# theori-io/nrsc5

Hardware: NVIDIA H100
Metric: cu8 I/Q Msamples/s (higher is better)
Workload: dtype u8/int16/f32

## Files before the change

### nrsc5_b200/csrc/front.cuh

```cuda
#pragma once
#include "pids_crc.cuh"
#include "common.cuh"
#include "fft.cuh"
#include "viterbi_pack.cuh"

namespace nb {

constexpr int FRONT_THREADS = 1024;
constexpr int TEAMS = FRONT_THREADS / 128;
constexpr int MAXREF = 15;
constexpr int IN_BYTES = 4 * NSYM + 28 + 16 + 16;
constexpr int IN_STRIDE = 8704;
constexpr int ACQ_TILE = 4096;

__device__ int g_dbg;

__constant__ int c_compat_mode[64];
__constant__ unsigned c_pn80[3];
__constant__ short c_bp_tap[32];

__device__ __forceinline__ float2 cmulf(float2 a, float2 b)
{
    return make_float2(a.x * b.x - a.y * b.y, a.x * b.y + a.y * b.x);
}
// ... 18 lines not shown
{
    StreamState &st = p.st[s];
    if (st.state == ns) return;
    if (st.state == ST_FINE) log_reserve(p, d, s, REC_LOST_SYNC, 0);
    if (ns == ST_FINE) {
        float fo = (float)(((double)st.prev_angle - 2 * M_PI * st.cfo) * 744187.5 / (2 * M_PI * NFFT));
        uint8_t *w = log_reserve(p, d, s, REC_SYNC, 8);
        if (w) {
            reinterpret_cast<float *>(w)[0] = fo;
            reinterpret_cast<int *>(w)[1] = st.psmi;
        }
    }
    st.state = ns;
}

constexpr int DEMOD_RUN = 17;
constexpr int TEAM_SMEM = IN_STRIDE + NSYM * (int)sizeof(short2);
struct DemodSmem {
    float2 buf[TEAMS][TEAM_SMEM / sizeof(float2)];
    float2 symphase[TEAMS];
};
static_assert(FFT_SMEM_ELEMS * sizeof(float2) <= TEAM_SMEM && TEAM_SMEM % 16 == 0, "a team's FFT buffer");
static_assert(DEMOD_RUN * FFT_THREADS >= NSYM && DEMOD_RUN % 2 == 1, "a symbol's runs");
struct PrepSmem {
    uint32_t words[ACQ_TILE + 40];
    short2 ytile[ACQ_TILE + 32];
    float2 sums[NSYM];
    float red_mag[FRONT_THREADS];
    int red_idx[FRONT_THREADS];
    float2 red_v[FRONT_THREADS];
};
constexpr int ACQ1_RUN = 3;
constexpr int ACQ1_WORDS = (NSYM + 38 + 3 + 3) / 4 * 4;
static_assert(ACQ1_RUN * FRONT_THREADS >= NSYM + 31 && ACQ1_RUN % 2 == 1, "a tile's runs");
struct Acq1Smem {
    uint32_t words[2][ACQ1_WORDS];
    short2 ytile[NSYM + 32];
    float2 ring[2][NSYM];
    float2 sums[NSYM];
    float2 shape[NCP];
    float red_mag[FRONT_THREADS];
    int red_idx[FRONT_THREADS];
    float2 red_v[FRONT_THREADS];
};
struct PidsSmem {
    int8_t vit[PIDS_LEN * 3];
    uint2 dec[PIDS_LEN + 64];
};
constexpr int ZS = 32;
constexpr int EQ_LD = BLK + 1;
constexpr int EQ_MAXPART = 12;
constexpr int EQ_ROWS = 2 * EQ_MAXPART * (PW - 1);
struct SyncSmem {
    float2 zref[BLK][ZS];
    float phs[BLK][ZS];
    float2 eph[2 * MAXREF][BLK];
    float smag[2 * MAXREF];
    float cfq[2 * MAXREF];
    union {
        float2 eq[EQ_ROWS][EQ_LD];
        struct {
            int offs[76][22];
            int verdict[76];
            int winner;
        } srch;
    };
    float wred[FRONT_THREADS / 32][2];
    float fb_w[2][MAXREF], fb_xy[2][MAXREF + 1];
    float4 rowc[EQ_ROWS];
    int ref_ok[2 * MAXREF], ref_bc[2 * MAXREF], ref_psmi[2 * MAXREF];
    float mult[2];
    float angle;
    int do_search;
};
struct FrontSmem {
    float2 tw[FFT_TW];
    float2 nco[NSYM];
    union {
        DemodSmem demod;
        PrepSmem prep;
        Acq1Smem acq1;
        SyncSmem sync;
        PidsSmem pidsq[16];
    } u;
};

__device__ void pids_decode_warp(const DevPtrs &p, const EngineDims &d, int s, int e, PidsSmem &sm, int lane)
{
    const StreamState &st = p.st[s];
    const int bc = st.pids_bc[e];
    const int8_t *pmall = p.pm + (size_t)s * 16 * PM_BLOCK;
    const int8_t PMV[20] = { 10, 2, 18, 6, 14, 8, 16, 0, 12, 4, 11, 3, 19, 7, 15, 9, 17, 1, 13, 5 };
    for (int o = lane; o < PIDS_LEN * 3; o += 32) {
        int8_t v = 0;
        if (o % 6 != 5) {
            unsigned i = (unsigned)bc * 200 + (unsigned)(o - o / 6);
            unsigned part = (unsigned)PMV[i % 20];
            unsigned block = i / 200;
            unsigned k = (i / 20) % 10 + P1_ENC / 320;
            unsigned row = (k * 11) % 32, col = (k * 11 + k / 288) % 36;
            v = pmall[(block * 32 + row) * 720 + part * 36 + col];
        }
        sm.vit[o] = v;
    }
    __syncwarp();
    const int l = lane & 15;
    VitHalf<false> vh;
    vh.init(l);
    vitc_run<false>(vh, sm.vit, PIDS_LEN, PIDS_LEN + 64, 0, PIDS_LEN + 64, 0, sm.dec, lane < 16, l);
    __syncwarp();
    int v = (short)(vh.E & 0xffff), state = 2 * l;
    const int w1 = (short)(vh.O & 0xffff);
    if (w1 > v) { v = w1; state = 2 * l + 1; }
    int v2 = (short)(vh.E >> 16), idx2 = 2 * l + 32;
    const int w3 = (short)(vh.O >> 16);
    if (w3 > v2) { v2 = w3; idx2 = 2 * l + 33; }
    if (v2 > v) { v = v2; state = idx2; }
#pragma unroll
    for (int o = 8; o; o >>= 1) {
        const int ov = __shfl_xor_sync(0xffffffffu, v, o, 16), oi = __shfl_xor_sync(0xffffffffu, state, o, 16);
        if (ov > v || (ov == v && oi < state)) { v = ov; state = oi; }
    }
    if (lane == 0) {
        uint8_t pk[10];
        for (int i = 0; i < 10; i++) pk[i] = 0;
        for (int q = PIDS_LEN + 63; q >= 0; q--) {
            if (q >= 32 && q < 32 + PIDS_LEN) {
                const int i = q - 32;
                const int bit = ((state >> 5) & 1) ^ (int)((c_pn80[i >> 5] >> (i & 31)) & 1u);
                pk[i >> 3] |= (uint8_t)(bit << (7 - (i & 7)));
// ... 373 lines not shown
        st.prev_angle = angle;
        sh_angle = angle;
    }
    __syncthreads();

    const int samperr = sh_samperr;
    const int adj = NSYM / 2 - samperr;
    if (adj != 0) {
        float *cp = p.cphase + (size_t)s * NFFT;
        for (int i = t; i < SIDE; i += FRONT_THREADS) {
            const int bl = LB0 + i, bu = UB1 - i;
            cp[bl] = (float)((double)cp[bl] - (double)(adj * (bl - NFFT / 2) * 2) * M_PI / NFFT);
            cp[bu] = (float)((double)cp[bu] - (double)(adj * (bu - NFFT / 2) * 2) * M_PI / NFFT);
        }
    }
    if (t == 0) {
        float angle = sh_angle;
        angle = (float)((double)angle - 2 * M_PI * st.cfo);
        const float pre = (float)(-adj) * angle / (float)NFFT;
        const float2 ph = cmulf(st.phase, cexp_j(pre));
        const float theta = angle / (float)NFFT;
        st.phase0 = ph;
        st.theta = theta;
        sh_theta = theta;
        st.blk_samperr = samperr;
        st.blk_state_in = state_in;
        double sn, cs;
        sincos((double)theta * (double)(NSYM * BLK), &sn, &cs);
        const float2 pe = cmulf(ph, make_float2((float)cs, (float)sn));
        const float nrm = sqrtf(pe.x * pe.x + pe.y * pe.y);
        st.phase = make_float2(pe.x / nrm, pe.y / nrm);
        uint8_t *w = log_reserve(p, d, s, REC_BLOCK, 32);
        if (w) {
            int *wi = reinterpret_cast<int *>(w);
            float *wf = reinterpret_cast<float *>(w);
            wi[0] = state_in; wi[1] = samperr; wf[2] = angle; wf[3] = ph.x; wf[4] = ph.y; wi[5] = st.cfo;
            wi[6] = (int)(unsigned)(st.start & 0xffffffffLL);
            wi[7] = (int)(st.start >> 32);
        }
    }
    __syncthreads();
    fill_nco(p, nco, sh_theta, t);
    __syncthreads();
    return true;
}

__device__ __forceinline__ float2 sample_q15(short2 h)
{
    const float sc = 1.0f / 32767.0f;
    return make_float2((float)h.x * sc, (float)h.y * -sc);
}

__device__ void front_demod(const DevPtrs &p, const EngineDims &d, int s, int sym, DemodSmem &sm, const float2 *nco,
                            const float2 *tw, int half, int tl, long long start, int samperr, float theta, float2 phase0)
{
    float2 *buf = sm.buf[half];
    uint8_t *in = reinterpret_cast<uint8_t *>(buf);
    const int bar = 1 + half;
    const long long base = start + samperr + (long long)NSYM * sym;
    const long long b0 = 4 * base - 28;
    const long long b0a = b0 & ~15LL;
    const int off = (int)(b0 - b0a);
    const uint8_t *iq = p.iq + (size_t)s * d.in_stride;
    bar_sync(bar);
    {
        const int nvec = (off + 4 * NSYM + 28 + 15) / 16;
        uint4 *dst = reinterpret_cast<uint4 *>(in);
        for (int v = tl; v < nvec; v += 128) {
            const long long a = b0a + 16LL * v;
            if (a >= 0) {
#if defined(NB_EMU)
                dst[v] = *reinterpret_cast<const uint4 *>(iq + a);
#else
                asm volatile("cp.async.cg.shared.global [%0], [%1], 16;" ::"r"((unsigned)__cvta_generic_to_shared(dst + v)), "l"(iq + a) : "memory");
#endif
            } else {
                dst[v] = make_uint4(0x7f7f7f7fu, 0x7f7f7f7fu, 0x7f7f7f7fu, 0x7f7f7f7fu);
            }
        }
#if !defined(NB_EMU)
        asm volatile("cp.async.commit_group;\n\tcp.async.wait_group 0;" ::: "memory");
#endif
    }
    if (tl == 0) {
        double sn, cs;
        sincos((double)theta * (double)(NSYM * sym), &sn, &cs);
        sm.symphase[half] = cmul(phase0, make_float2((float)cs, (float)sn));
    }
    bar_sync(bar);

    const uint32_t *sw = reinterpret_cast<const uint32_t *>(in + off);
    const short2 *y;
    if (d.cs16) {
        y = reinterpret_cast<const short2 *>(sw + 7);
    } else {
        short2 *yw = reinterpret_cast<short2 *>(in + IN_STRIDE);
        const int j0 = min(DEMOD_RUN * tl, NSYM - DEMOD_RUN);
        halfband_run<DEMOD_RUN>(sw + j0, yw + j0);
        y = yw;
        bar_sync(bar);
    }
    float2 v[16];
    v[0] = cmul(sample_q15(y[tl]), nco[tl]);
    if (tl < NCP) {
        const int j = NFFT + tl;
        v[0] = cadd(v[0], cmul(sample_q15(y[j]), nco[j]));
    }
#pragma unroll
    for (int n1 = 1; n1 < 16; n1++) {
        const int j = n1 * 128 + tl;
        v[n1] = cmul(sample_q15(y[j]), nco[j]);
    }
    bar_sync(bar);
    float2 out[2][8];
    fft2048_block<true>(v, out, buf, tw, tl, bar);
    const float2 sp = sm.symphase[half];

    float2 *dst = p.bins + ((size_t)s * BLK + sym) * NBINS;
#pragma unroll
    for (int h = 0; h < 2; h++) {
        const int q = tl + 128 * h;
        if (q >= 222) dst[q - 222] = cmul(out[h][5], sp);
        if (q <= 232) dst[q + 34] = cmul(out[h][6], sp);
        if (q >= 24) dst[q + 243] = cmul(out[h][1], sp);
        if (q <= 34) dst[q + 499] = cmul(out[h][2], sp);
    }
}

__device__ __forceinline__ int ref_bin(int slot)
{
    return slot < MAXREF ? LB0 + PW * slot : UB1 - PW * (slot - MAXREF);
}

__device__ __forceinline__ float atan2_short(float y, float x)
{
    const float ax = fabsf(x), ay = fabsf(y);
    const float mx = fmaxf(ax, ay), mn = fminf(ax, ay);
    const float t = mx > 0.f ? __fdividef(mn, mx) : 0.f;
    const float z = t * t;
    float p = 0.0028340641874819994f;
    p = __fmaf_rn(p, z, -0.016005029901862144f);
    p = __fmaf_rn(p, z, 0.042587608098983765f);
    p = __fmaf_rn(p, z, -0.07495445758104324f);
    p = __fmaf_rn(p, z, 0.10636754333972931f);
    p = __fmaf_rn(p, z, -0.14202570915222168f);
    p = __fmaf_rn(p, z, 0.19992484152317047f);
    p = __fmaf_rn(p, z, -0.3333306610584259f);
    p = __fmaf_rn(p, z, 1.0f);
    float r = p * t;
    if (ay > ax) r = 1.57079637f - r;
    if (x < 0.f) r = 3.14159274f - r;
    return copysignf(r, y);
}

__device__ __forceinline__ void costas_row(float2 *z, float *phs, int zs, float &cfreq, float &cphase, int cfo, float alpha, float beta, bool FAST)
{
    const unsigned pat_pos = (1u << 1) | (1u << 5) | (1u << 6) | (1u << 8) | (1u << 21);
    const unsigned pat_neg = (1u << 0) | (1u << 2) | (1u << 3) | (1u << 4) | (1u << 9) | (1u << 13) | (1u << 14) | (1u << 20) |
                             (1u << 22) | (1u << 31);
    const float cfo_freq = (float)(2 * M_PI * cfo * NCP / NFFT);
    const float PI_F = 3.14159274101257324f;
    const float TWO_PI_HI = 6.28318548202514648f, TWO_PI_LO = -1.74845553e-07f;
    float f = cfreq, ph = cphase;
#pragma unroll 1
    for (int n = 0; n < BLK; n++) {
        const float2 v = z[n * zs];
        float2 rot;
        if (FAST) {
            float sn, cs;
            __sincosf(-ph, &sn, &cs);
            rot = make_float2(cs, sn);
        } else {
            rot = cexp_j(-ph);
        }
        const float2 u = cmulf(v, rot);
        const float error = (FAST ? atan2_short((u.x * u.y) * 2.0f, u.x * u.x - u.y * u.y)
                                  : atan2f((u.x * u.y) * 2.0f, u.x * u.x - u.y * u.y)) * 0.5f;
        phs[n * zs] = ph;
// ... 18 lines not shown
    }
    cfreq = f;
    cphase = ph;
}

__device__ __forceinline__ int needle_bit(int n, unsigned rsid)
{
    const signed char base[BLK] = { 0, 1, 0, 0, 0, 1, 1, -1, 1, 0, 0, 0, -1, 0, 0, -1,
                                    -1, -1, -1, -1, 0, 1, 0, -1, -1, -1, -1, -1, -1, -1, -1, 0 };
    if (n == 10) return (int)(rsid >> 1);
    if (n == 11) return (int)((rsid >> 1) ^ (rsid & 1));
    return base[n];
}

__device__ int ref_find(const float2 *z, int zs, unsigned rsid)
{
    unsigned raw = 0;
    for (int n = 0; n < BLK; n++)
        if (!(z[n * zs].x <= 0)) raw |= 1u << n;
    for (int pass = 0; pass < 2; pass++) {
        for (int n = 0; n < BLK; n++) {
            int i;
            for (i = 0; i < BLK; i++) {
                const int nb_ = needle_bit(i, rsid);
                if (nb_ < 0) continue;
                if (nb_ != (int)((raw >> ((n + i) & 31)) & 1)) break;
            }
            if (i == BLK) return n;
        }
        raw = ~raw;
    }
    return -1;
}

__device__ __forceinline__ float half_pi_wrap(float a, float b)
{
    float dd = a - b;
    while ((double)dd > M_PI / 2) dd = (float)((double)dd - M_PI);
    while ((double)dd < -M_PI / 2) dd = (float)((double)dd + M_PI);
    return dd;
}

__device__ __forceinline__ int8_t soft_demap(float x, float mult)
{
    const float v = fmaxf(fminf(x, 1.0f), -1.0f) * mult;
    int r = __float2int_rz(v);
    const float f = v - (float)r;
    if (f >= 0.5f) r++;
    else if (f <= -0.5f) r--;
    return (int8_t)r;
}

template <bool CL>
__device__ void front_sync(const DevPtrs &p, const EngineDims &d, int s, SyncSmem &sm, int t)
{
    StreamState &st = p.st[s];
    float *cfreq = p.cfreq + (size_t)s * NFFT;
    float *cphase = p.cphase + (size_t)s * NFFT;
    float2 *bins = p.bins + (size_t)s * BLK * NBINS;
    auto ldbin = [](const float2 *q) -> float2 { return CL ? __ldcg(q) : *q; };
    const float loop_bw = 0.05f, damping = 0.70710678f;
    const float denom = 1 + (2 * damping * loop_bw) + (loop_bw * loop_bw);
    const float alpha = (4 * damping * loop_bw) / denom, beta = (4 * loop_bw * loop_bw) / denom;

    int ppb = partitions_per_band(st.psmi);
    int nref = ppb + 1;
    long long sy0 = clock64();
    const bool sy_on = st.state == ST_FINE;
    auto sylap = [&](int k) {
        if (t == 0 && sy_on) {
            const long long c1 = clock64();
            st.sy_cyc[k] += (unsigned long long)(c1 - sy0);
            sy0 = c1;
        }
    };
    auto stage_eq = [&](int first, int stride) {
        const int rows = min(ppb, EQ_MAXPART) * (PW - 1), rows2 = 2 * rows;
#pragma unroll 4
        for (int idx = first; idx < rows2 * BLK; idx += stride) {
            const int n = idx / rows2, r = idx - n * rows2;
            const int sb = r >= rows, rr = sb ? r - rows : r;
            const int i = rr / (PW - 1), k = rr - i * (PW - 1) + 1;
            const int ci = sb == 0 ? PW * i + k : (NBINS - 1 - PW) - PW * i + k;
            sm.eq[r][n] = ldbin(&bins[(size_t)n * NBINS + ci]);
        }
    };
    const bool pre_staged = st.state == ST_FINE && !(g_dbg & 1);
    for (int i = t; i < ZS * BLK; i += FRONT_THREADS) {
        const int slot = i & (ZS - 1), n = i / ZS;
        const int ii = slot < MAXREF ? slot : slot - MAXREF;
        if (slot < 2 * MAXREF && ii < nref) sm.zref[n][slot] = ldbin(&bins[(size_t)n * NBINS + compact_of_bin(ref_bin(slot))]);
    }
    __syncthreads();
    sylap(0);
    if (t < 2 * MAXREF) {
        const int i = t < MAXREF ? t : t - MAXREF;
        if (i < nref) {
            const int b = ref_bin(t);
            float f = cfreq[b], ph = cphase[b];
            costas_row(&sm.zref[0][t], &sm.phs[0][t], ZS, f, ph, 0, alpha, beta, !(g_dbg & 2));
            cfreq[b] = f;
            cphase[b] = ph;
            sm.cfq[t] = f;
        }
    } else if (t >= 32 && pre_staged) {
        stage_eq(t - 32, FRONT_THREADS - 32);
    }
    __syncthreads();
    sylap(1);

    if (st.state == ST_COARSE) {
        if (t < 2 * MAXREF) {
            const int i = t < MAXREF ? t : t - MAXREF;
            sm.ref_ok[t] = 0;
            if (i < nref) {
                const float2 *z = &sm.zref[0][t];
                const unsigned rsid = (unsigned)(30 - i) & 3;
                bool ok = true;
                unsigned raw = 0;
                for (int n = 0; n < BLK; n++) {
                    const int nbit = needle_bit(n, rsid);
                    const int pos = z[n * ZS].x > 0 ? 1 : 0;
                    if (nbit >= 0 && nbit != pos) ok = false;
                    if (!(z[n * ZS].x <= 0)) raw |= 1u << n;
                }
                const unsigned dd = raw ^ (raw << 1);
                auto bit = [&](int n) { return (dd >> n) & 1u; };
                sm.ref_ok[t] = ok;
                sm.ref_bc[t] = (int)(bit(16) << 3 | bit(17) << 2 | bit(18) << 1 | bit(19));
                sm.ref_psmi[t] = (int)(bit(25) << 5 | bit(26) << 4 | bit(27) << 3 | bit(28) << 2 | bit(29) << 1 | bit(30));
            }
        }
        __syncthreads();
        if (t == 0) {
            unsigned good = 0;
            for (int r = 0; r < 2 * MAXREF; r++)
                if (sm.ref_ok[r]) good++;
            sm.do_search = 0;
            if (good >= 4) {
                int mbc = -1, mps = -1;
                for (int v = 0; v < 16; v++) {
                    unsigned nbc = 0, nps = 0;
                    for (int r = 0; r < 2 * MAXREF; r++) {
                        if (!sm.ref_ok[r]) continue;
                        nbc += sm.ref_bc[r] == v;
                        nps += sm.ref_psmi[r] == v;
                    }
                    if (nbc > good / 2) mbc = v;
                    if (nps > good / 2) mps = v;
                }
                if (mbc >= 0 && mps >= 0) {
                    st.bc = mbc;
                    st.psmi = mps;
                    set_state(p, d, s, ST_FINE);
                    l2_enqueue(st, d.l2, 0u, 0, 0);
                    st.started_pm = 0;
                    st.px_total[0] = st.px_total[1] = 0;
                    st.px_started[0] = st.px_started[1] = 0;
                }
            } else if (st.cfo_wait == 0) {
                sm.do_search = 1;
            } else {
                st.cfo_wait--;
            }
        }
        __syncthreads();
        if (sm.do_search) {
            for (int i = t; i < ZS * BLK; i += FRONT_THREADS) {
                const int slot = i & (ZS - 1), n = i / ZS;
                const int ii = slot < MAXREF ? slot : slot - MAXREF;
                if (slot < 2 * MAXREF && ii < nref) bins[(size_t)n * NBINS + compact_of_bin(ref_bin(slot))] = sm.zref[n][slot];
            }
            for (int i = t; i < 76 * 22; i += FRONT_THREADS) sm.srch.offs[i / 22][i % 22] = -1;
            __syncthreads();
            constexpr int SB_BINS = 2 * PW * 2 + 10 * PW;
            constexpr int NSB = 2 * SB_BINS;
            float2 *snap = p.tbuf + (size_t)s * NACQ;
            float *sphs = reinterpret_cast<float *>(p.ydec + (size_t)s * NACQ);
            float fs[4], phsn[4];
            int cfo_of[4], nq = 0, ci = -1, b = 0;
            if (t < NSB) {
                const int upper = t >= SB_BINS;
                b = upper ? (UB1 - 10 * PW - 2 * PW) + (t - SB_BINS) : (LB0 - 2 * PW) + t;
                ci = compact_of_bin(b);
                float f = cfreq[b], ph = cphase[b];
                int ref_i[4];
                for (int step = 0; step <= 10; step++) {
                    const int i = upper ? step : 10 - step;
                    const int cfo = upper ? b - UB1 + PW * i : b - LB0 - PW * i;
                    if (cfo >= -2 * PW && cfo < 2 * PW && nq < 4) {
                        ref_i[nq] = i;
                        cfo_of[nq] = cfo;
                        nq++;
                    }
                }
                for (int q = 0; q < nq; q++) {
                    const int i = ref_i[q], cfo = cfo_of[q];
                    float2 *row = snap + (size_t)q * BLK * NSB + t;
                    const float2 *src = q ? snap + (size_t)(q - 1) * BLK * NSB + t : nullptr;
                    for (int n = 0; n < BLK; n++)
                        row[(size_t)n * NSB] = q ? src[(size_t)n * NSB]
                                                 : (ci >= 0 ? ldbin(&bins[(size_t)n * NBINS + ci]) : make_float2(0.f, 0.f));
                    costas_row(row, sphs + t, NSB, f, ph, cfo, alpha, beta, false);
                    sm.srch.offs[cfo + 2 * PW][2 * i + upper] = ref_find(row, NSB, (unsigned)(30 - i) & 3);
                    for (int n = 0; n < BLK; n++)
                        row[(size_t)n * NSB] = cmulf(row[(size_t)n * NSB], cexp_j(sphs[(size_t)n * NSB + t]));
                    fs[q] = f;
                    phsn[q] = ph;
                }
            }
            __syncthreads();
            if (t < 76) {
                int best = -1;
                unsigned bestn = 0;
                for (int k = 0; k < BLK; k++) {
                    unsigned nv = 0;
                    for (int r = 0; r < 22; r++) nv += sm.srch.offs[t][r] == k;
                    if (nv > bestn) { best = k; bestn = nv; }
                }
                sm.srch.verdict[t] = (best >= 0 && bestn >= 3) ? best : -1;
            }
            __syncthreads();
            if (t == 0) {
                int win = 1 << 20;
                for (int c = 0; c < 76; c++)
                    if (sm.srch.verdict[c] >= 0) { win = c - 2 * PW; break; }
                sm.srch.winner = win;
                if (win < (1 << 20)) {
                    st.keep_extra = ((BLK - sm.srch.verdict[win + 2 * PW]) % BLK) * NSYM;
                    st.cfo += win;
                    st.cfo_wait = 8;
                }
            }
            __syncthreads();
            if (t < NSB) {
                const int win = sm.srch.winner;
                int q = -1;
                for (int k = 0; k < nq; k++)
                    if (cfo_of[k] <= win) q = k;
                if (q >= 0) {
                    cfreq[b] = fs[q];
                    cphase[b] = phsn[q];
                    if (ci >= 0) {
                        const float2 *row = snap + (size_t)q * BLK * NSB + t;
                        for (int n = 0; n < BLK; n++) bins[(size_t)n * NBINS + ci] = row[(size_t)n * NSB];
                    }
                }
            }
        }
        __syncthreads();
    }

    if (st.state == ST_FINE) {
        if (t < 2 * MAXREF) {
            const int i = t < MAXREF ? t : t - MAXREF;
            if (i < nref) {
                float sum = 0;
                for (int n = 0; n < BLK; n++) sum += fabsf(sm.zref[n][t].x);
                sm.smag[t] = sum / BLK;
            }
        }
        for (int i = t; i < 2 * MAXREF * BLK; i += FRONT_THREADS) {
            const int slot = i >> 5, n = i & 31;
            const int ii = slot < MAXREF ? slot : slot - MAXREF;
            if (ii < nref) sm.eph[slot][n] = cexp_j(sm.phs[n][slot]);
        }
        if (t >= FRONT_THREADS - 32) {
            const int lane = t & 31;
            if (lane < ppb) {
                sm.fb_w[0][lane] = half_pi_wrap(sm.phs[0][lane], sm.phs[0][lane + 1]);
                sm.fb_w[1][lane] = half_pi_wrap(sm.phs[0][MAXREF + lane + 1], sm.phs[0][MAXREF + lane]);
            }
            if (lane <= ppb) {
                sm.fb_xy[0][lane] = (float)(LB0 + PW * lane - NFFT / 2) * sm.cfq[lane];
                sm.fb_xy[1][lane] = (float)(UB1 - PW * lane - NFFT / 2) * sm.cfq[MAXREF + lane];
            }
            __syncwarp();
            if (lane == 31) {
                float samperr = 0, angle = 0, sum_xy = 0, sum_x2 = 0;
                for (int i = 0; i < ppb; i++) {
                    samperr += sm.fb_w[0][i];
                    samperr += sm.fb_w[1][i];
                }
                const double inv_2pi = 1.0 / (2 * M_PI);
                samperr = (float)((double)(samperr / (float)(ppb * 2) * (float)NFFT / (float)PW) * inv_2pi);
                for (int i = 0; i <= ppb; i++) {
                    float x;
                    x = (float)(LB0 + PW * i - NFFT / 2);
                    angle += sm.cfq[i]; sum_xy += sm.fb_xy[0][i]; sum_x2 += x * x;
                    x = (float)(UB1 - PW * i - NFFT / 2);
                    angle += sm.cfq[MAXREF + i]; sum_xy += sm.fb_xy[1][i]; sum_x2 += x * x;
                }
                samperr = (float)((double)samperr - (double)((sum_xy / sum_x2) * (float)NFFT) * inv_2pi * BLK);
                st.samperr = (int)roundf(samperr);
                angle /= (float)((ppb + 1) * 2);
                st.angle = angle;
                sm.angle = angle;
            }
        }
        __syncthreads();
        if (t < 2 * MAXREF) {
            const int i = t < MAXREF ? t : t - MAXREF;
            if (i < nref) cfreq[ref_bin(t)] = sm.cfq[t] - sm.angle;
        }
        const int bc = st.bc;
        int8_t *pm = p.pm + ((size_t)s * 16 + bc) * PM_BLOCK;
        const int rows = min(ppb, EQ_MAXPART) * (PW - 1), rows2 = 2 * rows;
        sylap(2);
        if (!pre_staged) stage_eq(t, FRONT_THREADS);
        for (int r = t; r < rows2; r += FRONT_THREADS) {
            const int sb = r >= rows, rr = sb ? r - rows : r;
            const int i = rr / (PW - 1), k = rr - i * (PW - 1) + 1;
            int slot_lo, slot_hi;
            if (sb == 0) { slot_lo = i; slot_hi = i + 1; }
            else { slot_lo = MAXREF + i + 1; slot_hi = MAXREF + i; }
            sm.rowc[r] = make_float4((float)k * sm.smag[slot_hi], (float)(PW - k) * sm.smag[slot_lo],
                                     __int_as_float(slot_hi), __int_as_float(slot_lo));
        }
        __syncthreads();
        sylap(3);
        float e_lb = 0.f, e_ub = 0.f;
        if (ppb > EQ_MAXPART) {
            const int xrows = (ppb - EQ_MAXPART) * (PW - 1);
            for (int idx = t; idx < 2 * xrows * BLK; idx += FRONT_THREADS) {
                const int r = idx >> 5, n = idx & (BLK - 1);
                const int sb = r >= xrows, rr = sb ? r - xrows : r;
                const int i = EQ_MAXPART + rr / (PW - 1), k = rr % (PW - 1) + 1;
                const int ci = sb == 0 ? PW * i + k : (NBINS - 1 - PW) - PW * i + k;
                const int slot_lo = sb == 0 ? i : MAXREF + i + 1, slot_hi = sb == 0 ? i + 1 : MAXREF + i;
                const float fa = (float)k * sm.smag[slot_hi], fb = (float)(PW - k) * sm.smag[slot_lo];
                const float2 up = sm.eph[slot_hi][n], lp = sm.eph[slot_lo][n];
                const float c = fa * up.x + fb * lp.x, dd = fa * up.y + fb * lp.y;
                const float rden = __fdividef(19.0f, c * c + dd * dd);
                const float2 C = make_float2((c + dd) * rden, (c - dd) * rden);
                const float2 v = cmulf(ldbin(&bins[(size_t)n * NBINS + ci]), C);
                bins[(size_t)n * NBINS + ci] = v;
                const float dx = (v.x >= 0 ? 1.0f : -1.0f) - v.x, dy = (v.y >= 0 ? 1.0f : -1.0f) - v.y;
                const float e = dx * dx + dy * dy;
                if (sb) e_ub += e;
                else e_lb += e;
            }
        }
        for (int idx = t; idx < rows2 * BLK; idx += FRONT_THREADS) {
            const int r = idx >> 5, n = idx & (BLK - 1);
            const float4 rc = sm.rowc[r];
            const float fa = rc.x, fb = rc.y;
            const float2 up = sm.eph[__float_as_int(rc.z)][n], lp = sm.eph[__float_as_int(rc.w)][n];
            const float c = fa * up.x + fb * lp.x, dd = fa * up.y + fb * lp.y;
            const float rden = __fdividef(19.0f, c * c + dd * dd);
            const float2 C = make_float2((c + dd) * rden, (c - dd) * rden);
            const float2 v = cmulf(sm.eq[r][n], C);
            sm.eq[r][n] = v;
            const float dx = (v.x >= 0 ? 1.0f : -1.0f) - v.x, dy = (v.y >= 0 ? 1.0f : -1.0f) - v.y;
            const float e = dx * dx + dy * dy;
            if (r >= rows) e_ub += e;
            else e_lb += e;
        }
#pragma unroll
        for (int o = 16; o; o >>= 1) {
            e_lb += __shfl_xor_sync(0xffffffffu, e_lb, o);
            e_ub += __shfl_xor_sync(0xffffffffu, e_ub, o);
        }
        if ((t & 31) == 0) { sm.wred[t >> 5][0] = e_lb; sm.wred[t >> 5][1] = e_ub; }
        __syncthreads();
        float e_sb[2] = { 0.f, 0.f };
        if (t < 32) {
            float a = sm.wred[t][0], b = sm.wred[t][1];
#pragma unroll
            for (int o = 16; o; o >>= 1) {
                a += __shfl_xor_sync(0xffffffffu, a, o);
                b += __shfl_xor_sync(0xffffffffu, b, o);
            }
            if (t == 0) {
                e_sb[0] = a;
                e_sb[1] = b;
                const float mer_lb = 2.0f * BLK * (float)(ppb * 18) / a, mer_ub = 2.0f * BLK * (float)(ppb * 18) / b;
                sm.mult[0] = fmaxf(fminf(mer_lb * 10, 127.0f), 1.0f);
                sm.mult[1] = fmaxf(fminf(mer_ub * 10, 127.0f), 1.0f);
            }
        }
        __syncthreads();
        sylap(4);
        for (int item = t; item < BLK * 20 * 9; item += FRONT_THREADS) {
            const int n = item / 180, rem = item - n * 180;
            const int part = rem / 9, c4 = rem - part * 9;
            const int sb = part >= 10;
            const int r = (sb ? rows + (19 - part) * (PW - 1) : part * (PW - 1)) + 2 * c4;
            const float mult = sm.mult[sb];
            const float2 a = sm.eq[r][n], b = sm.eq[r + 1][n];
            const unsigned w = (unsigned)(uint8_t)soft_demap(a.x, mult) | ((unsigned)(uint8_t)soft_demap(a.y, mult) << 8) |
                               ((unsigned)(uint8_t)soft_demap(b.x, mult) << 16) | ((unsigned)(uint8_t)soft_demap(b.y, mult) << 24);
            *reinterpret_cast<uint32_t *>(pm + n * 720 + part * 36 + 4 * c4) = w;
        }
        const int cm = c_compat_mode[st.psmi & 63];
        const bool has_px1 = cm == 2 || cm == 3 || cm == 11;
        const int eqparts = rows / (PW - 1);
        auto px_demap = [&](int8_t *ring, long long T, int nq, int base, bool lower_scale_only) {
            const int per_sym = nq * 36;
            for (int item = t; item < BLK * nq * 9; item += FRONT_THREADS) {
                const int n = item / (nq * 9), rem = item - n * (nq * 9);
                const int q = rem / 9, c4 = rem - q * 9;
                const int sb = q >= nq / 2;
                const int i = nq == 2 ? base : ((q == 0 || q == 3) ? base : base + 1);
                float2 a, b;
                if (i < eqparts) {
                    const int r = (sb ? rows : 0) + i * (PW - 1) + 2 * c4;
                    a = sm.eq[r][n];
                    b = sm.eq[r + 1][n];
                } else {
                    const int ci = (sb == 0 ? PW * i : (NBINS - 1 - PW) - PW * i) + 1 + 2 * c4;
                    a = ldbin(&bins[(size_t)n * NBINS + ci]);
                    b = ldbin(&bins[(size_t)n * NBINS + ci + 1]);
                }
                const float mult = sm.mult[lower_scale_only ? 0 : sb];
                const unsigned w = (unsigned)(uint8_t)soft_demap(a.x, mult) | ((unsigned)(uint8_t)soft_demap(a.y, mult) << 8) |
                                   ((unsigned)(uint8_t)soft_demap(b.x, mult) << 16) | ((unsigned)(uint8_t)soft_demap(b.y, mult) << 24);
                const long long pos = (T + n * per_sym + q * 36 + 4 * c4) % PX_RING;
                *reinterpret_cast<uint32_t *>(ring + pos) = w;
            }
        };
        if (has_px1 && (st.px_started[0] || (bc & 1) == 0))
            px_demap(p.px_ring[0] + (size_t)s * PX_RING, st.px_total[0], cm == 2 ? 2 : 4, 10, false);
        if (cm == 11 && (st.px_started[1] || (bc & 1) == 0))
            px_demap(p.px_ring[1] + (size_t)s * PX_RING, st.px_total[1], 4, 12, true);
        __syncthreads();
        if (t == 0) {
            st.err_lb += e_sb[0];
            st.err_ub += e_sb[1];
            if (++st.mer_cnt == 16) {
                const float signal = (float)(2 * BLK * (ppb * 18) * st.mer_cnt);
                uint8_t *w = log_reserve(p, d, s, REC_MER, 8);
                if (w) {
                    reinterpret_cast<float *>(w)[0] = 10 * log10f(signal / st.err_lb);
                    reinterpret_cast<float *>(w)[1] = 10 * log10f(signal / st.err_ub);
                }
                st.mer_cnt = 0;
                st.err_lb = 0;
                st.err_ub = 0;
            }
        }
        if (d.emit_soft) {
            __shared__ uint8_t *sh_w;
            __syncthreads();
            if (t == 0) {
                sh_w = log_reserve(p, d, s, REC_SOFT_PM, 4 + PM_BLOCK);
                if (sh_w) *reinterpret_cast<uint32_t *>(sh_w) = (uint32_t)bc;
            }
            __syncthreads();
            if (sh_w)
                for (int o = t; o < PM_BLOCK; o += FRONT_THREADS) sh_w[4 + o] = (uint8_t)pm[o];
            __syncthreads();
        }
        if (t == 0) {
            uint8_t *w = log_reserve(p, d, s, REC_PIDS, 11);
            const int e = st.pids_pending;
            st.pids_rec[e] = w ? (unsigned)(w - (p.log + (size_t)s * d.log_cap)) : 0xffffffffu;
            st.pids_bc[e] = bc;
            st.pids_pending = e + 1;
            if (bc == 0) st.started_pm = 1;
            unsigned lost_slot = 0xffffffffu;
            if (st.started_pm && bc == 15) {
                const unsigned len0 = st.log_len;
                uint8_t *bw = log_reserve(p, d, s, REC_BER, 4);
                uint8_t *fw = bw ? log_reserve(p, d, s, REC_FRAME, 8 + P1_LEN / 8) : nullptr;
                if (!fw) { st.log_len = len0; bw = nullptr; }
                st.p1_rec = (bw && fw) ? (unsigned)(bw - (p.log + (size_t)s * d.log_cap)) : 0xffffffffu;
                if (fw) {
                    reinterpret_cast<uint32_t *>(fw)[0] = 0;
                    reinterpret_cast<uint32_t *>(fw)[1] = P1_LEN;
                    uint8_t *lw = log_reserve(p, d, s, REC_PAD, 0);
                    if (lw) lost_slot = (unsigned)(lw - 8 - (p.log + (size_t)s * d.log_cap));
                }
                st.p1_lost_rec = lost_slot;
                l2_enqueue(st, d.l2, st.p1_rec != 0xffffffffu ? st.p1_rec + 4 + 8 + 8 : 0xffffffffu, 0, P1_LEN);
                st.p1_ready = 1;
            }
#pragma unroll
            for (int g = 0; g < PX_GROUPS; g++) {
                const PxGroup x = px_group(g);
                if (!(x.modes >> cm & 1)) continue;
                if ((bc & 1) == 0) st.px_started[x.ring] = 1;
                if (!st.px_started[x.ring]) continue;
                st.px_total[x.ring] += x.len;
                const long long k0 = st.px_total[x.ring] - 2 * x.len;
                if ((bc & 1) && k0 >= 32 * x.len && st.xq_pending[g] < P3_SLOTS) {
                    uint8_t *fw = log_reserve(p, d, s, REC_FRAME, 8 + x.len / 8);
                    const int e = st.xq_pending[g];
                    st.xq_k0[g][e] = k0;
                    st.xq_rec[g][e] = fw ? (unsigned)(fw - (p.log + (size_t)s * d.log_cap)) : 0xffffffffu;
                    if (fw) {
                        reinterpret_cast<uint32_t *>(fw)[0] = x.lc;
                        reinterpret_cast<uint32_t *>(fw)[1] = x.len;
                    }
                    l2_enqueue(st, d.l2, fw ? st.xq_rec[g][e] + 8 : 0xffffffffu, x.lc, x.len);
                    st.xq_pending[g] = e + 1;
                }
            }
            if (lost_slot != 0xffffffffu && st.log_len == lost_slot + 8) {
                st.log_len = lost_slot;
                st.p1_lost_rec = 0xffffffffu;
            }
            st.bc = (bc + 1) % 16;
        }
    }
    __syncthreads();
    if (t == 0) {
        const int keep = NSYM + (NSYM / 2 - st.blk_samperr) + st.keep_extra;
        st.keep_extra = 0;
        st.start += NACQ - keep;
        st.blocks_done++;
    }
    sylap(5);
}

__device__ __forceinline__ void cluster_barrier()
{
#if defined(NB_EMU)
#else
    asm volatile("barrier.cluster.arrive.release.aligned;\n\tbarrier.cluster.wait.acquire.aligned;" ::: "memory");
#endif
}

template <bool CL>
__global__ void __launch_bounds__(FRONT_THREADS, 1) k_stream(DevPtrs p, EngineDims d, int max_blocks, int last_pass)
{
#if defined(NB_EMU)
    unsigned char *front_smem_raw = emu::dyn_smem();
#else
    extern __shared__ __align__(16) unsigned char front_smem_raw[];
#endif
    FrontSmem &sm = *reinterpret_cast<FrontSmem *>(front_smem_raw);
    const int t = threadIdx.x, team = t >> 7, tl = t & 127;
    const int C = CL ? d.cluster : 1;
    const int s = (int)blockIdx.x / C, rank = (int)blockIdx.x % C;
    StreamState &st = p.st[s];
    for (int i = t; i < FFT_TW; i += FRONT_THREADS) sm.tw[i] = __ldg(&p.twid[i]);
    __syncthreads();

    const bool owner = !CL || rank == 0;
    if (max_blocks > 16) max_blocks = 16;
    if (owner && t == 0) {
        for (int g = 0; g < PX_GROUPS; g++) st.xq_pending[g] = 0;
    }
    __syncthreads();
    for (int nb = 0;; nb++) {
        long long c0 = clock64();
        auto lap = [&](int ph) {
            if (owner && t == 0) {
                const long long c1 = clock64();
                st.ph_cyc[ph] += (unsigned long long)(c1 - c0);
                st.ph_n[ph]++;
                c0 = c1;
            }
        };
        int mode = 0;
        if (!CL) {
            if (nb < max_blocks && !st.p1_ready) mode = front_prep_single(p, d, s, sm.u.acq1, sm.nco, t) ? 1 : 0;
            if (mode == 0) break;
        } else {
            if (owner) {
                if (nb < max_blocks && !st.p1_ready) mode = front_prep_begin(p, d, s, t);
                if (mode == 1) front_prep_finish(p, d, s, sm.u.prep, sm.nco, t, 1);
            }
            if (owner && t == 0) {
                st.blk_go = mode;
                __threadfence();
            }
            cluster_barrier();
            if (!owner) mode = __ldcg(&st.blk_go);
            if (mode == 0) break;
            if (mode == 2) {
                front_acq_tiles(p, d, s, sm.u.prep, t, rank, C);
                __threadfence();
                cluster_barrier();
                front_acq_corr(p, s, t, rank, C);
                __threadfence();
                cluster_barrier();
                if (owner) {
                    front_prep_finish(p, d, s, sm.u.prep, sm.nco, t, 2);
                    __threadfence();
                }
                cluster_barrier();
            }
        }
        lap(st.blk_state_in == ST_FINE ? 2 : 1);
        const long long start = CL ? __ldcg(&st.start) : st.start;
        const int samperr = CL ? __ldcg(&st.blk_samperr) : st.blk_samperr;
        const float theta = CL ? __ldcg(&st.theta) : st.theta;
        const float2 phase0 = CL ? __ldcg(&st.phase0) : st.phase0;
        if (CL && !owner) {
            fill_nco(p, sm.nco, theta, t);
            __syncthreads();
        }
#pragma unroll 1
        for (int pass = 0; pass < BLK / (TEAMS * C); pass++)
            front_demod(p, d, s, (pass * C + rank) * TEAMS + team, sm.u.demod, sm.nco, sm.tw, team, tl, start, samperr, theta, phase0);
        if (CL) {
            __threadfence();
            cluster_barrier();
        }
        if (CL && !owner) continue;
        __syncthreads();
        lap(3);
        front_sync<CL>(p, d, s, sm.u.sync, t);
        __syncthreads();
        lap(st.blk_state_in == ST_FINE ? 4 : 5);
    }
    if (CL && !owner) return;
    __syncthreads();
    if (st.pids_pending) {
        const long long c0 = clock64();
        front_pids_flush(p, d, s, sm.u.pidsq, t);
        if (t == 0) {
            st.ph_cyc[0] += (unsigned long long)(clock64() - c0);
            st.ph_n[0]++;
        }
    }
    if (t == 0) {
        StreamBrief b;
        b.start = st.start;
        b.state = st.state;
        b.bc = st.bc;
        b.p1_ready = st.p1_ready;
        b.pad_ = 0;
        p.brief[s] = b;
        const long long avail = *reinterpret_cast<volatile long long *>(&st.in_avail);
        if (last_pass && avail >= 2 * (st.start + NACQ)) atomicAdd(&p.ctl->more, 1u);
    }
}

}
```

Before: 155,800.

## Capture reference bins during demod and overlap sync feedback with soft demapping

Moves the zref pilot buffer out of the sync union into persistent shared memory and fills it directly from the FFT output in demod, using precomputed slot and mask tables, so the non-cluster path skips re-reading reference bins from global memory. The sync stage is restructured: the smag average moves into the Costas loop threads, the MER multipliers are computed per warp with shuffles instead of a shared broadcast and barrier, and the samperr/angle feedback warp runs concurrently with the soft-demap threads. Soft-log copying and px state are staged so several __syncthreads are removed, and the stage_eq index math is made incremental. The cost is more shared memory and more complex warp-role splitting.

Result: faster. 161,900, median of 6 (+3.9%).

```diff
diff --git a/nrsc5_b200/csrc/front.cuh b/nrsc5_b200/csrc/front.cuh
--- a/nrsc5_b200/csrc/front.cuh
+++ b/nrsc5_b200/csrc/front.cuh
@@ -94,7 +94,6 @@
 constexpr int EQ_MAXPART = 12;
 constexpr int EQ_ROWS = 2 * EQ_MAXPART * (PW - 1);
 struct SyncSmem {
-    float2 zref[BLK][ZS];
     float phs[BLK][ZS];
     float2 eph[2 * MAXREF][BLK];
     float smag[2 * MAXREF];
@@ -111,13 +110,17 @@
     float fb_w[2][MAXREF], fb_xy[2][MAXREF + 1];
     float4 rowc[EQ_ROWS];
     int ref_ok[2 * MAXREF], ref_bc[2 * MAXREF], ref_psmi[2 * MAXREF];
-    float mult[2];
-    float angle;
+    bool px_on[2];
+    long long px_T[2];
+    uint8_t *soft_w;
     int do_search;
 };
 struct FrontSmem {
     float2 tw[FFT_TW];
     float2 nco[NSYM];
+    float2 zref[BLK][ZS];
+    signed char ref_slot[NBINS + 2];
+    uint8_t ref_mask[128];
     union {
         DemodSmem demod;
         PrepSmem prep;
@@ -597,7 +600,8 @@
 }
 
 __device__ void front_demod(const DevPtrs &p, const EngineDims &d, int s, int sym, DemodSmem &sm, const float2 *nco,
-                            const float2 *tw, int half, int tl, long long start, int samperr, float theta, float2 phase0)
+                            const float2 *tw, float2 (*zref)[ZS], const signed char *ref_slot, const uint8_t *ref_mask,
+                            int half, int tl, long long start, int samperr, float theta, float2 phase0)
 {
     float2 *buf = sm.buf[half];
     uint8_t *in = reinterpret_cast<uint8_t *>(buf);
@@ -662,13 +666,19 @@
     const float2 sp = sm.symphase[half];
 
     float2 *dst = p.bins + ((size_t)s * BLK + sym) * NBINS;
+    float2 *zr = zref[sym];
+    const unsigned mask = ref_mask[tl];
+    auto put = [&](int c, float2 v, int bit) {
+        dst[c] = v;
+        if (mask & (1u << bit)) zr[ref_slot[c]] = v;
+    };
 #pragma unroll
     for (int h = 0; h < 2; h++) {
         const int q = tl + 128 * h;
-        if (q >= 222) dst[q - 222] = cmul(out[h][5], sp);
-        if (q <= 232) dst[q + 34] = cmul(out[h][6], sp);
-        if (q >= 24) dst[q + 243] = cmul(out[h][1], sp);
-        if (q <= 34) dst[q + 499] = cmul(out[h][2], sp);
+        if (q >= 222) put(q - 222, cmul(out[h][5], sp), 4 * h);
+        if (q <= 232) put(q + 34, cmul(out[h][6], sp), 4 * h + 1);
+        if (q >= 24) put(q + 243, cmul(out[h][1], sp), 4 * h + 2);
+        if (q <= 34) put(q + 499, cmul(out[h][2], sp), 4 * h + 3);
     }
 }
 
@@ -793,7 +803,7 @@
 }
 
 template <bool CL>
-__device__ void front_sync(const DevPtrs &p, const EngineDims &d, int s, SyncSmem &sm, int t)
+__device__ void front_sync(const DevPtrs &p, const EngineDims &d, int s, SyncSmem &sm, float2 (*zref)[ZS], int t)
 {
     StreamState &st = p.st[s];
     float *cfreq = p.cfreq + (size_t)s * NFFT;
@@ -817,32 +827,41 @@
     };
     auto stage_eq = [&](int first, int stride) {
         const int rows = min(ppb, EQ_MAXPART) * (PW - 1), rows2 = 2 * rows;
+        const int dn = stride / rows2, dr = stride - dn * rows2;
+        int n = first / rows2, r = first - n * rows2;
 #pragma unroll 4
-        for (int idx = first; idx < rows2 * BLK; idx += stride) {
-            const int n = idx / rows2, r = idx - n * rows2;
+        for (; n < BLK;) {
             const int sb = r >= rows, rr = sb ? r - rows : r;
-            const int i = rr / (PW - 1), k = rr - i * (PW - 1) + 1;
-            const int ci = sb == 0 ? PW * i + k : (NBINS - 1 - PW) - PW * i + k;
+            const int i = rr / (PW - 1);
+            const int ci = sb == 0 ? rr + i + 1 : (NBINS - PW) + rr - (2 * PW - 1) * i;
             sm.eq[r][n] = ldbin(&bins[(size_t)n * NBINS + ci]);
+            r += dr;
+            n += dn;
+            if (r >= rows2) { r -= rows2; n++; }
         }
     };
     const bool pre_staged = st.state == ST_FINE && !(g_dbg & 1);
-    for (int i = t; i < ZS * BLK; i += FRONT_THREADS) {
-        const int slot = i & (ZS - 1), n = i / ZS;
-        const int ii = slot < MAXREF ? slot : slot - MAXREF;
-        if (slot < 2 * MAXREF && ii < nref) sm.zref[n][slot] = ldbin(&bins[(size_t)n * NBINS + compact_of_bin(ref_bin(slot))]);
-    }
-    __syncthreads();
+    if (CL) {
+        for (int i = t; i < ZS * BLK; i += FRONT_THREADS) {
+            const int slot = i & (ZS - 1), n = i / ZS;
+            const int ii = slot < MAXREF ? slot : slot - MAXREF;
+            if (slot < 2 * MAXREF && ii < nref) zref[n][slot] = ldbin(&bins[(size_t)n * NBINS + compact_of_bin(ref_bin(slot))]);
+        }
+        __syncthreads();
+    }
     sylap(0);
     if (t < 2 * MAXREF) {
         const int i = t < MAXREF ? t : t - MAXREF;
         if (i < nref) {
             const int b = ref_bin(t);
             float f = cfreq[b], ph = cphase[b];
-            costas_row(&sm.zref[0][t], &sm.phs[0][t], ZS, f, ph, 0, alpha, beta, !(g_dbg & 2));
+            costas_row(&zref[0][t], &sm.phs[0][t], ZS, f, ph, 0, alpha, beta, !(g_dbg & 2));
             cfreq[b] = f;
             cphase[b] = ph;
             sm.cfq[t] = f;
+            float sum = 0;
+            for (int n = 0; n < BLK; n++) sum += fabsf(zref[n][t].x);
+            sm.smag[t] = sum / BLK;
         }
     } else if (t >= 32 && pre_staged) {
         stage_eq(t - 32, FRONT_THREADS - 32);
@@ -855,7 +874,7 @@
             const int i = t < MAXREF ? t : t - MAXREF;
             sm.ref_ok[t] = 0;
             if (i < nref) {
-                const float2 *z = &sm.zref[0][t];
+                const float2 *z = &zref[0][t];
                 const unsigned rsid = (unsigned)(30 - i) & 3;
                 bool ok = true;
                 unsigned raw = 0;
@@ -910,7 +929,7 @@
             for (int i = t; i < ZS * BLK; i += FRONT_THREADS) {
                 const int slot = i & (ZS - 1), n = i / ZS;
                 const int ii = slot < MAXREF ? slot : slot - MAXREF;
-                if (slot < 2 * MAXREF && ii < nref) bins[(size_t)n * NBINS + compact_of_bin(ref_bin(slot))] = sm.zref[n][slot];
+                if (slot < 2 * MAXREF && ii < nref) bins[(size_t)n * NBINS + compact_of_bin(ref_bin(slot))] = zref[n][slot];
             }
             for (int i = t; i < 76 * 22; i += FRONT_THREADS) sm.srch.offs[i / 22][i % 22] = -1;
             __syncthreads();
@@ -993,62 +1012,14 @@
     }
 
     if (st.state == ST_FINE) {
-        if (t < 2 * MAXREF) {
-            const int i = t < MAXREF ? t : t - MAXREF;
-            if (i < nref) {
-                float sum = 0;
-                for (int n = 0; n < BLK; n++) sum += fabsf(sm.zref[n][t].x);
-                sm.smag[t] = sum / BLK;
-            }
-        }
         for (int i = t; i < 2 * MAXREF * BLK; i += FRONT_THREADS) {
             const int slot = i >> 5, n = i & 31;
             const int ii = slot < MAXREF ? slot : slot - MAXREF;
             if (ii < nref) sm.eph[slot][n] = cexp_j(sm.phs[n][slot]);
         }
-        if (t >= FRONT_THREADS - 32) {
-            const int lane = t & 31;
-            if (lane < ppb) {
-                sm.fb_w[0][lane] = half_pi_wrap(sm.phs[0][lane], sm.phs[0][lane + 1]);
-                sm.fb_w[1][lane] = half_pi_wrap(sm.phs[0][MAXREF + lane + 1], sm.phs[0][MAXREF + lane]);
-            }
-            if (lane <= ppb) {
-                sm.fb_xy[0][lane] = (float)(LB0 + PW * lane - NFFT / 2) * sm.cfq[lane];
-                sm.fb_xy[1][lane] = (float)(UB1 - PW * lane - NFFT / 2) * sm.cfq[MAXREF + lane];
-            }
-            __syncwarp();
-            if (lane == 31) {
-                float samperr = 0, angle = 0, sum_xy = 0, sum_x2 = 0;
-                for (int i = 0; i < ppb; i++) {
-                    samperr += sm.fb_w[0][i];
-                    samperr += sm.fb_w[1][i];
-                }
-                const double inv_2pi = 1.0 / (2 * M_PI);
-                samperr = (float)((double)(samperr / (float)(ppb * 2) * (float)NFFT / (float)PW) * inv_2pi);
-                for (int i = 0; i <= ppb; i++) {
-                    float x;
-                    x = (float)(LB0 + PW * i - NFFT / 2);
-                    angle += sm.cfq[i]; sum_xy += sm.fb_xy[0][i]; sum_x2 += x * x;
-                    x = (float)(UB1 - PW * i - NFFT / 2);
-                    angle += sm.cfq[MAXREF + i]; sum_xy += sm.fb_xy[1][i]; sum_x2 += x * x;
-                }
-                samperr = (float)((double)samperr - (double)((sum_xy / sum_x2) * (float)NFFT) * inv_2pi * BLK);
-                st.samperr = (int)roundf(samperr);
-                angle /= (float)((ppb + 1) * 2);
-                st.angle = angle;
-                sm.angle = angle;
-            }
-        }
-        __syncthreads();
-        if (t < 2 * MAXREF) {
-            const int i = t < MAXREF ? t : t - MAXREF;
-            if (i < nref) cfreq[ref_bin(t)] = sm.cfq[t] - sm.angle;
-        }
         const int bc = st.bc;
         int8_t *pm = p.pm + ((size_t)s * 16 + bc) * PM_BLOCK;
         const int rows = min(ppb, EQ_MAXPART) * (PW - 1), rows2 = 2 * rows;
-        sylap(2);
-        if (!pre_staged) stage_eq(t, FRONT_THREADS);
         for (int r = t; r < rows2; r += FRONT_THREADS) {
             const int sb = r >= rows, rr = sb ? r - rows : r;
             const int i = rr / (PW - 1), k = rr - i * (PW - 1) + 1;
@@ -1057,6 +1028,16 @@
             else { slot_lo = MAXREF + i + 1; slot_hi = MAXREF + i; }
             sm.rowc[r] = make_float4((float)k * sm.smag[slot_hi], (float)(PW - k) * sm.smag[slot_lo],
                                      __int_as_float(slot_hi), __int_as_float(slot_lo));
+        }
+        sylap(2);
+        if (!pre_staged) stage_eq(t, FRONT_THREADS);
+        const int cm = c_compat_mode[st.psmi & 63];
+        const bool has_px1 = cm == 2 || cm == 3 || cm == 11;
+        if (t == 0) {
+            sm.px_on[0] = has_px1 && (st.px_started[0] || (bc & 1) == 0);
+            sm.px_on[1] = cm == 11 && (st.px_started[1] || (bc & 1) == 0);
+            sm.px_T[0] = st.px_total[0];
+            sm.px_T[1] = st.px_total[1];
         }
         __syncthreads();
         sylap(3);
@@ -1104,68 +1085,101 @@
         }
         if ((t & 31) == 0) { sm.wred[t >> 5][0] = e_lb; sm.wred[t >> 5][1] = e_ub; }
         __syncthreads();
-        float e_sb[2] = { 0.f, 0.f };
-        if (t < 32) {
-            float a = sm.wred[t][0], b = sm.wred[t][1];
+        float mult[2], e_sb[2];
+        {
+            const int lane = t & 31;
+            float a = sm.wred[lane][0], b = sm.wred[lane][1];
 #pragma unroll
             for (int o = 16; o; o >>= 1) {
                 a += __shfl_xor_sync(0xffffffffu, a, o);
                 b += __shfl_xor_sync(0xffffffffu, b, o);
             }
-            if (t == 0) {
-                e_sb[0] = a;
-                e_sb[1] = b;
-                const float mer_lb = 2.0f * BLK * (float)(ppb * 18) / a, mer_ub = 2.0f * BLK * (float)(ppb * 18) / b;
-                sm.mult[0] = fmaxf(fminf(mer_lb * 10, 127.0f), 1.0f);
-                sm.mult[1] = fmaxf(fminf(mer_ub * 10, 127.0f), 1.0f);
-            }
-        }
-        __syncthreads();
+            e_sb[0] = __shfl_sync(0xffffffffu, a, 0);
+            e_sb[1] = __shfl_sync(0xffffffffu, b, 0);
+            const float mer_lb = 2.0f * BLK * (float)(ppb * 18) / e_sb[0], mer_ub = 2.0f * BLK * (float)(ppb * 18) / e_sb[1];
+            mult[0] = fmaxf(fminf(mer_lb * 10, 127.0f), 1.0f);
+            mult[1] = fmaxf(fminf(mer_ub * 10, 127.0f), 1.0f);
+        }
         sylap(4);
-        for (int item = t; item < BLK * 20 * 9; item += FRONT_THREADS) {
-            const int n = item / 180, rem = item - n * 180;
-            const int part = rem / 9, c4 = rem - part * 9;
-            const int sb = part >= 10;
-            const int r = (sb ? rows + (19 - part) * (PW - 1) : part * (PW - 1)) + 2 * c4;
-            const float mult = sm.mult[sb];
-            const float2 a = sm.eq[r][n], b = sm.eq[r + 1][n];
-            const unsigned w = (unsigned)(uint8_t)soft_demap(a.x, mult) | ((unsigned)(uint8_t)soft_demap(a.y, mult) << 8) |
-                               ((unsigned)(uint8_t)soft_demap(b.x, mult) << 16) | ((unsigned)(uint8_t)soft_demap(b.y, mult) << 24);
-            *reinterpret_cast<uint32_t *>(pm + n * 720 + part * 36 + 4 * c4) = w;
-        }
-        const int cm = c_compat_mode[st.psmi & 63];
-        const bool has_px1 = cm == 2 || cm == 3 || cm == 11;
-        const int eqparts = rows / (PW - 1);
-        auto px_demap = [&](int8_t *ring, long long T, int nq, int base, bool lower_scale_only) {
-            const int per_sym = nq * 36;
-            for (int item = t; item < BLK * nq * 9; item += FRONT_THREADS) {
-                const int n = item / (nq * 9), rem = item - n * (nq * 9);
-                const int q = rem / 9, c4 = rem - q * 9;
-                const int sb = q >= nq / 2;
-                const int i = nq == 2 ? base : ((q == 0 || q == 3) ? base : base + 1);
-                float2 a, b;
-                if (i < eqparts) {
-                    const int r = (sb ? rows : 0) + i * (PW - 1) + 2 * c4;
-                    a = sm.eq[r][n];
-                    b = sm.eq[r + 1][n];
-                } else {
-                    const int ci = (sb == 0 ? PW * i : (NBINS - 1 - PW) - PW * i) + 1 + 2 * c4;
-                    a = ldbin(&bins[(size_t)n * NBINS + ci]);
-                    b = ldbin(&bins[(size_t)n * NBINS + ci + 1]);
-                }
-                const float mult = sm.mult[lower_scale_only ? 0 : sb];
-                const unsigned w = (unsigned)(uint8_t)soft_demap(a.x, mult) | ((unsigned)(uint8_t)soft_demap(a.y, mult) << 8) |
-                                   ((unsigned)(uint8_t)soft_demap(b.x, mult) << 16) | ((unsigned)(uint8_t)soft_demap(b.y, mult) << 24);
-                const long long pos = (T + n * per_sym + q * 36 + 4 * c4) % PX_RING;
-                *reinterpret_cast<uint32_t *>(ring + pos) = w;
-            }
-        };
-        if (has_px1 && (st.px_started[0] || (bc & 1) == 0))
-            px_demap(p.px_ring[0] + (size_t)s * PX_RING, st.px_total[0], cm == 2 ? 2 : 4, 10, false);
-        if (cm == 11 && (st.px_started[1] || (bc & 1) == 0))
-            px_demap(p.px_ring[1] + (size_t)s * PX_RING, st.px_total[1], 4, 12, true);
-        __syncthreads();
-        if (t == 0) {
+        constexpr int DEMAP_T0 = 64;
+        if (t >= DEMAP_T0) {
+            const int td = t - DEMAP_T0;
+            constexpr int DSTRIDE = FRONT_THREADS - DEMAP_T0;
+            for (int item = td; item < BLK * 20 * 9; item += DSTRIDE) {
+                const int n = item / 180, rem = item - n * 180;
+                const int part = rem / 9, c4 = rem - part * 9;
+                const int sb = part >= 10;
+                const int r = (sb ? rows + (19 - part) * (PW - 1) : part * (PW - 1)) + 2 * c4;
+                const float ml = mult[sb];
+                const float2 a = sm.eq[r][n], b = sm.eq[r + 1][n];
+                const unsigned w = (unsigned)(uint8_t)soft_demap(a.x, ml) | ((unsigned)(uint8_t)soft_demap(a.y, ml) << 8) |
+                                   ((unsigned)(uint8_t)soft_demap(b.x, ml) << 16) | ((unsigned)(uint8_t)soft_demap(b.y, ml) << 24);
+                *reinterpret_cast<uint32_t *>(pm + n * 720 + part * 36 + 4 * c4) = w;
+            }
+            const int eqparts = rows / (PW - 1);
+            auto px_demap = [&](int8_t *ring, long long T, int nq, int base, bool lower_scale_only) {
+                const int per_sym = nq * 36;
+                for (int item = td; item < BLK * nq * 9; item += DSTRIDE) {
+                    const int n = item / (nq * 9), rem = item - n * (nq * 9);
+                    const int q = rem / 9, c4 = rem - q * 9;
+                    const int sb = q >= nq / 2;
+                    const int i = nq == 2 ? base : ((q == 0 || q == 3) ? base : base + 1);
+                    float2 a, b;
+                    if (i < eqparts) {
+                        const int r = (sb ? rows : 0) + i * (PW - 1) + 2 * c4;
+                        a = sm.eq[r][n];
+                        b = sm.eq[r + 1][n];
+                    } else {
+                        const int ci = (sb == 0 ? PW * i : (NBINS - 1 - PW) - PW * i) + 1 + 2 * c4;
+                        a = ldbin(&bins[(size_t)n * NBINS + ci]);
+                        b = ldbin(&bins[(size_t)n * NBINS + ci + 1]);
+                    }
+                    const float ml = mult[lower_scale_only ? 0 : sb];
+                    const unsigned w = (unsigned)(uint8_t)soft_demap(a.x, ml) | ((unsigned)(uint8_t)soft_demap(a.y, ml) << 8) |
+                                       ((unsigned)(uint8_t)soft_demap(b.x, ml) << 16) | ((unsigned)(uint8_t)soft_demap(b.y, ml) << 24);
+                    const long long pos = (T + n * per_sym + q * 36 + 4 * c4) % PX_RING;
+                    *reinterpret_cast<uint32_t *>(ring + pos) = w;
+                }
+            };
+            if (sm.px_on[0]) px_demap(p.px_ring[0] + (size_t)s * PX_RING, sm.px_T[0], cm == 2 ? 2 : 4, 10, false);
+            if (sm.px_on[1]) px_demap(p.px_ring[1] + (size_t)s * PX_RING, sm.px_T[1], 4, 12, true);
+        } else if (t >= 32) {
+            const int lane = t & 31;
+            if (lane < ppb) {
+                sm.fb_w[0][lane] = half_pi_wrap(sm.phs[0][lane], sm.phs[0][lane + 1]);
+                sm.fb_w[1][lane] = half_pi_wrap(sm.phs[0][MAXREF + lane + 1], sm.phs[0][MAXREF + lane]);
+            }
+            if (lane <= ppb) {
+                sm.fb_xy[0][lane] = (float)(LB0 + PW * lane - NFFT / 2) * sm.cfq[lane];
+                sm.fb_xy[1][lane] = (float)(UB1 - PW * lane - NFFT / 2) * sm.cfq[MAXREF + lane];
+            }
+            __syncwarp();
+            float fb_angle = 0;
+            if (lane == 31) {
+                float samperr = 0, angle = 0, sum_xy = 0, sum_x2 = 0;
+                for (int i = 0; i < ppb; i++) {
+                    samperr += sm.fb_w[0][i];
+                    samperr += sm.fb_w[1][i];
+                }
+                const double inv_2pi = 1.0 / (2 * M_PI);
+                samperr = (float)((double)(samperr / (float)(ppb * 2) * (float)NFFT / (float)PW) * inv_2pi);
+                for (int i = 0; i <= ppb; i++) {
+                    float x;
+                    x = (float)(LB0 + PW * i - NFFT / 2);
+                    angle += sm.cfq[i]; sum_xy += sm.fb_xy[0][i]; sum_x2 += x * x;
+                    x = (float)(UB1 - PW * i - NFFT / 2);
+                    angle += sm.cfq[MAXREF + i]; sum_xy += sm.fb_xy[1][i]; sum_x2 += x * x;
+                }
+                samperr = (float)((double)samperr - (double)((sum_xy / sum_x2) * (float)NFFT) * inv_2pi * BLK);
+                st.samperr = (int)roundf(samperr);
+                angle /= (float)((ppb + 1) * 2);
+                st.angle = angle;
+                fb_angle = angle;
+            }
+            fb_angle = __shfl_sync(0xffffffffu, fb_angle, 31);
+            const int i = lane < MAXREF ? lane : lane - MAXREF;
+            if (lane < 2 * MAXREF && i < nref) cfreq[ref_bin(lane)] = sm.cfq[lane] - fb_angle;
+        } else if (t == 0) {
             st.err_lb += e_sb[0];
             st.err_ub += e_sb[1];
             if (++st.mer_cnt == 16) {
@@ -1179,20 +1193,10 @@
                 st.err_lb = 0;
                 st.err_ub = 0;
             }
-        }
-        if (d.emit_soft) {
-            __shared__ uint8_t *sh_w;
-            __syncthreads();
-            if (t == 0) {
-                sh_w = log_reserve(p, d, s, REC_SOFT_PM, 4 + PM_BLOCK);
-                if (sh_w) *reinterpret_cast<uint32_t *>(sh_w) = (uint32_t)bc;
-            }
-            __syncthreads();
-            if (sh_w)
-                for (int o = t; o < PM_BLOCK; o += FRONT_THREADS) sh_w[4 + o] = (uint8_t)pm[o];
-            __syncthreads();
-        }
-        if (t == 0) {
+            if (d.emit_soft) {
+                sm.soft_w = log_reserve(p, d, s, REC_SOFT_PM, 4 + PM_BLOCK);
+                if (sm.soft_w) *reinterpret_cast<uint32_t *>(sm.soft_w) = (uint32_t)bc;
+            }
             uint8_t *w = log_reserve(p, d, s, REC_PIDS, 11);
             const int e = st.pids_pending;
             st.pids_rec[e] = w ? (unsigned)(w - (p.log + (size_t)s * d.log_cap)) : 0xffffffffu;
@@ -1243,8 +1247,10 @@
             }
             st.bc = (bc + 1) % 16;
         }
-    }
-    __syncthreads();
+        __syncthreads();
+        if (d.emit_soft && sm.soft_w)
+            for (int o = t; o < PM_BLOCK; o += FRONT_THREADS) sm.soft_w[4 + o] = (uint8_t)pm[o];
+    }
     if (t == 0) {
         const int keep = NSYM + (NSYM / 2 - st.blk_samperr) + st.keep_extra;
         st.keep_extra = 0;
@@ -1276,6 +1282,18 @@
     const int s = (int)blockIdx.x / C, rank = (int)blockIdx.x % C;
     StreamState &st = p.st[s];
     for (int i = t; i < FFT_TW; i += FRONT_THREADS) sm.tw[i] = __ldg(&p.twid[i]);
+    for (int c = t; c < NBINS; c += FRONT_THREADS)
+        sm.ref_slot[c] = c < SIDE ? (c % PW == 0 ? c / PW : -1) : ((NBINS - 1 - c) % PW == 0 ? MAXREF + (NBINS - 1 - c) / PW : -1);
+    if (t < 128) {
+        unsigned m = 0;
+        for (int h = 0; h < 2; h++) {
+            const int q = t + 128 * h;
+            const int c[4] = { q >= 222 ? q - 222 : -1, q <= 232 ? q + 34 : -1, q >= 24 ? q + 243 : -1, q <= 34 ? q + 499 : -1 };
+            for (int k = 0; k < 4; k++)
+                if (c[k] >= 0 && (c[k] < SIDE ? c[k] % PW == 0 : (NBINS - 1 - c[k]) % PW == 0)) m |= 1u << (4 * h + k);
+        }
+        sm.ref_mask[t] = (uint8_t)m;
+    }
     __syncthreads();
 
     const bool owner = !CL || rank == 0;
@@ -1335,7 +1353,7 @@
         }
 #pragma unroll 1
         for (int pass = 0; pass < BLK / (TEAMS * C); pass++)
-            front_demod(p, d, s, (pass * C + rank) * TEAMS + team, sm.u.demod, sm.nco, sm.tw, team, tl, start, samperr, theta, phase0);
+            front_demod(p, d, s, (pass * C + rank) * TEAMS + team, sm.u.demod, sm.nco, sm.tw, sm.zref, sm.ref_slot, sm.ref_mask, team, tl, start, samperr, theta, phase0);
         if (CL) {
             __threadfence();
             cluster_barrier();
@@ -1343,7 +1361,7 @@
         if (CL && !owner) continue;
         __syncthreads();
         lap(3);
-        front_sync<CL>(p, d, s, sm.u.sync, t);
+        front_sync<CL>(p, d, s, sm.u.sync, sm.zref, t);
         __syncthreads();
         lap(st.blk_state_in == ST_FINE ? 4 : 5);
     }
```
